# mvenouziou/Boosted_DETR

Measured on AMD Instinct MI355X. Metric: images/sec training step (fwd+matcher+loss+bwd), 640x640 N=100, higher is better.
Workload: dtype f32 (conv/GEMM products as 3 split-f16 [fwd] / split-bf16 [grad] MFMA products, f32 accumulate)

## Files before the change

### boosted_detr_amd/csrc/attention.hip

```cpp
#include "common.h"
#include "p16.h"
#include <stdlib.h>

namespace bdgemm { int gemm_mode(); }

namespace {

typedef unsigned int u32x4 __attribute__((ext_vector_type(4)));
typedef unsigned int u32x2 __attribute__((ext_vector_type(2)));
typedef short s16x4 __attribute__((ext_vector_type(4)));
typedef __bf16 abf16x8 __attribute__((ext_vector_type(8)));
typedef _Float16 af16x8 __attribute__((ext_vector_type(8)));
enum { AR_FP32 = 0, AR_BF16 = 1, AR_F16 = 2 };

constexpr int AD = 32;
constexpr int ALD = AD + 4;
constexpr int CH = 64;
constexpr int COLS_PER_BLOCK = 128;
#ifndef BDETR_ATTN_PF
#define BDETR_ATTN_PF 1
#endif
constexpr int APF = BDETR_ATTN_PF;

constexpr float LOG2E = 1.4426950408889634f, LN2 = 0.6931471805599453f;
__device__ __forceinline__ float exp2_fast(float x) { return __builtin_amdgcn_exp2f(x); }

__device__ __forceinline__ int crow(int e, int lh) { return (e & 3) + 8 * (e >> 2) + 4 * lh; }

struct ChunkRegs { f32x4 v[2]; };
__device__ __forceinline__ ChunkRegs fetch_chunk(const float* __restrict__ base, int64_t stride, int r0, int n) {
    ChunkRegs c;
#pragma unroll
    for (int p = 0; p < 2; ++p) {
        const int v = threadIdx.x + 256 * p;
        const int row = v >> 3, c4 = v & 7;
        const int rr = min(r0 + row, n - 1);
        f32x4 val = *reinterpret_cast<const f32x4*>(base + (int64_t)rr * stride + 4 * c4);
        if (r0 + row >= n) val = f32x4{0.f, 0.f, 0.f, 0.f};
        c.v[p] = val;
    }
    return c;
}
__device__ __forceinline__ void store_chunk(float* __restrict__ lds, const ChunkRegs& c) {
#pragma unroll
    for (int p = 0; p < 2; ++p) {
        const int v = threadIdx.x + 256 * p;
        *reinterpret_cast<f32x4*>(lds + (v >> 3) * ALD + 4 * (v & 7)) = c.v[p];
    }
}

__device__ __forceinline__ void load_col_regs(float (&r)[16], const float* __restrict__ base, int64_t stride, int col, bool ok, int lh) {
#pragma unroll
    for (int c = 0; c < 4; ++c) {
        f32x4 v = {0.f, 0.f, 0.f, 0.f};
        if (ok) v = *reinterpret_cast<const f32x4*>(base + (int64_t)col * stride + 16 * lh + 4 * c);
#pragma unroll
        for (int e = 0; e < 4; ++e) r[4 * c + e] = v[e];
    }
}

__device__ __forceinline__ f32x16 row_times_col(const float* __restrict__ sR, int t, const float (&creg)[16], int li, int lh) {
    f32x16 acc;
#pragma unroll
    for (int e = 0; e < 16; ++e) acc[e] = 0.f;
    f32x4 a[4];
#pragma unroll
    for (int c = 0; c < 4; ++c) a[c] = *reinterpret_cast<const f32x4*>(sR + (32 * t + li) * ALD + 16 * lh + 4 * c);
#pragma unroll
    for (int s = 0; s < 16; ++s) acc = __builtin_amdgcn_mfma_f32_32x32x2f32(a[s >> 2][s & 3], creg[s], acc, 0, 0, 0);
    return acc;
}

__device__ __forceinline__ void accumulate_rt_tile(f32x16& acc, const float* __restrict__ sR, int t, const f32x16& tile, int li, int lh) {
#pragma unroll
    for (int e = 0; e < 16; ++e) {
        const float a = sR[(32 * t + crow(e, lh)) * ALD + li];
        acc = __builtin_amdgcn_mfma_f32_32x32x2f32(a, tile[e], acc, 0, 0, 0);
    }
}

constexpr int IMG_PLANE = CH * 64, IMG_BYTES = 2 * IMG_PLANE;
constexpr int SMEM_BYTES = IMG_BYTES > CH * ALD * 4 ? IMG_BYTES : CH * ALD * 4;

template <int AR>
__device__ __forceinline__ void split2(float x0, float x1, unsigned& hi, unsigned& lo) {
    if (AR == AR_F16) p16_split2_f16(x0, x1, hi, lo); else p16_split2_bf16(x0, x1, hi, lo);
}
template <int AR>
__device__ __forceinline__ f32x16 mfma3(const u32x4& ah, const u32x4& al, const u32x4& bh, const u32x4& bl, f32x16 acc) {
    if (AR == AR_F16) {
#define H8(v) __builtin_bit_cast(af16x8, v)
        acc = __builtin_amdgcn_mfma_f32_32x32x16_f16(H8(al), H8(bh), acc, 0, 0, 0);
        acc = __builtin_amdgcn_mfma_f32_32x32x16_f16(H8(ah), H8(bl), acc, 0, 0, 0);
        acc = __builtin_amdgcn_mfma_f32_32x32x16_f16(H8(ah), H8(bh), acc, 0, 0, 0);
#undef H8
    } else {
#define B8(v) __builtin_bit_cast(abf16x8, v)
        acc = __builtin_amdgcn_mfma_f32_32x32x16_bf16(B8(al), B8(bh), acc, 0, 0, 0);
        acc = __builtin_amdgcn_mfma_f32_32x32x16_bf16(B8(ah), B8(bl), acc, 0, 0, 0);
        acc = __builtin_amdgcn_mfma_f32_32x32x16_bf16(B8(ah), B8(bh), acc, 0, 0, 0);
#undef B8
    }
    return acc;
}
template <int AR>
__device__ __forceinline__ void store_chunk_split(unsigned char* __restrict__ img, const ChunkRegs& c) {
#pragma unroll
    for (int p = 0; p < 2; ++p) {
        const int v = threadIdx.x + 256 * p, row = v >> 3, c4 = v & 7;
        unsigned h0, l0, h1, l1;
        split2<AR>(c.v[p][0], c.v[p][1], h0, l0);
        split2<AR>(c.v[p][2], c.v[p][3], h1, l1);
        const int off = row * 64 + (((c4 >> 1) ^ ((row >> 2) & 3)) << 4) + ((c4 & 1) << 3);
        *reinterpret_cast<u32x2*>(img + off) = u32x2{h0, h1};
        *reinterpret_cast<u32x2*>(img + IMG_PLANE + off) = u32x2{l0, l1};
    }
}
struct ColFrag { u32x4 h[2], l[2]; };
template <int AR>
__device__ __forceinline__ ColFrag col_frag(const float (&r)[16]) {
    ColFrag f;
#pragma unroll
    for (int s2 = 0; s2 < 2; ++s2)
#pragma unroll
        for (int e = 0; e < 4; ++e) { unsigned h, l; split2<AR>(r[8 * s2 + 2 * e], r[8 * s2 + 2 * e + 1], h, l); f.h[s2][e] = h; f.l[s2][e] = l; }
    return f;
}
template <int AR>
__device__ __forceinline__ f32x16 row_times_col_split(const unsigned char* __restrict__ img, int t, const ColFrag& c, int li, int lh) {
    f32x16 acc;
#pragma unroll
    for (int e = 0; e < 16; ++e) acc[e] = 0.f;
    const int row = 32 * t + li;
#pragma unroll
    for (int s2 = 0; s2 < 2; ++s2) {
        const int off = row * 64 + (((2 * lh + s2) ^ ((row >> 2) & 3)) << 4);
        const u32x4 ah = *reinterpret_cast<const u32x4*>(img + off), al = *reinterpret_cast<const u32x4*>(img + IMG_PLANE + off);
        acc = mfma3<AR>(ah, al, c.h[s2], c.l[s2], acc);
    }
    return acc;
}
template <int AR>
__device__ __forceinline__ void accumulate_rt_tile_split(f32x16& acc, const unsigned char* __restrict__ img, int t, const f32x16& tile, int lane) {
    const int lh = lane >> 5, g16 = (lane >> 4) & 1, q = (lane >> 2) & 3, p = lane & 3;
#pragma unroll
    for (int s2 = 0; s2 < 2; ++s2) {
        u32x4 bh, bl;
#pragma unroll
        for (int e = 0; e < 4; ++e) { unsigned h, l; split2<AR>(tile[8 * s2 + 2 * e], tile[8 * s2 + 2 * e + 1], h, l); bh[e] = h; bl[e] = l; }
        u32x2 ah2[2], al2[2];
#pragma unroll
        for (int jj = 0; jj < 2; ++jj) {
            const int row = 32 * t + 16 * s2 + 8 * jj + 4 * lh + q;
            const int off = row * 64 + ((((2 * g16) + (p >> 1)) ^ ((row >> 2) & 3)) << 4) + ((p & 1) << 3);
            ah2[jj] = __builtin_bit_cast(u32x2, __builtin_amdgcn_ds_read_tr16_b64_v4i16((__attribute__((address_space(3))) s16x4*)(img + off)));
            al2[jj] = __builtin_bit_cast(u32x2, __builtin_amdgcn_ds_read_tr16_b64_v4i16((__attribute__((address_space(3))) s16x4*)(img + IMG_PLANE + off)));
        }
        const u32x4 ah = {ah2[0][0], ah2[0][1], ah2[1][0], ah2[1][1]}, al = {al2[0][0], al2[0][1], al2[1][0], al2[1][1]};
        acc = mfma3<AR>(ah, al, bh, bl, acc);
    }
}

template <int AR> struct ColOperand { float r[16]; ColFrag f; };
template <int AR>
__device__ __forceinline__ void chunk_store(unsigned char* smem, const ChunkRegs& c) {
    if constexpr (AR == AR_FP32) store_chunk(reinterpret_cast<float*>(smem), c); else store_chunk_split<AR>(smem, c);
}
template <int AR>
__device__ __forceinline__ f32x16 rows_x_col(const unsigned char* smem, int t, const ColOperand<AR>& c, int li, int lh) {
    if constexpr (AR == AR_FP32) return row_times_col(reinterpret_cast<const float*>(smem), t, c.r, li, lh);
    else return row_times_col_split<AR>(smem, t, c.f, li, lh);
}
template <int AR>
__device__ __forceinline__ void rowsT_x_tile(f32x16& acc, const unsigned char* smem, int t, const f32x16& tile, int lane) {
    if constexpr (AR == AR_FP32) accumulate_rt_tile(acc, reinterpret_cast<const float*>(smem), t, tile, lane & 31, lane >> 5);
    else accumulate_rt_tile_split<AR>(acc, smem, t, tile, lane);
}
template <int AR>
__device__ __forceinline__ void col_operand(ColOperand<AR>& c, const float* __restrict__ base, int64_t stride, int col, bool ok, int lh) {
    load_col_regs(c.r, base, stride, col, ok, lh);
    if constexpr (AR != AR_FP32) c.f = col_frag<AR>(c.r);
}

template <int AR>
__global__ __launch_bounds__(256) void attn_fwd_kernel(const float* __restrict__ q, const float* __restrict__ k, const float* __restrict__ v,
                                                       float* __restrict__ o, float* __restrict__ lse,
                                                       int h, int nq, int nk, float scale) {
    __shared__ __attribute__((aligned(16))) unsigned char sK[SMEM_BYTES];
    __shared__ __attribute__((aligned(16))) unsigned char sV[SMEM_BYTES];
    const int b = blockIdx.z, head = blockIdx.y;
    const int lane = threadIdx.x & 63, wave = threadIdx.x >> 6, li = lane & 31, lh = lane >> 5;
    const int64_t D = (int64_t)h * AD;
    const int qi = blockIdx.x * COLS_PER_BLOCK + wave * 32 + li;
    const bool qok = qi < nq;
    ColOperand<AR> qr;
    col_operand<AR>(qr, q + (int64_t)b * nq * D + head * AD, D, qi, qok, lh);
    const float* kbase = k + (int64_t)b * nk * D + head * AD;
    const float* vbase = v + (int64_t)b * nk * D + head * AD;

    f32x16 oacc;
#pragma unroll
    for (int e = 0; e < 16; ++e) oacc[e] = 0.f;
    float m = -INFINITY, l = 0.f;

    const float scale2 = scale * LOG2E;
    const bool wave_active = blockIdx.x * COLS_PER_BLOCK + wave * 32 < nq;
    ChunkRegs ck[APF], cv[APF];
#pragma unroll
    for (int p = 0; p < APF; ++p) {
        ck[p] = ChunkRegs{}; cv[p] = ChunkRegs{};
        if (p * CH < nk) { ck[p] = fetch_chunk(kbase, D, p * CH, nk); cv[p] = fetch_chunk(vbase, D, p * CH, nk); }
    }
    for (int c0 = 0; c0 < nk; c0 += CH) {
        __syncthreads();
        chunk_store<AR>(sK, ck[0]);
        chunk_store<AR>(sV, cv[0]);
        __syncthreads();
#pragma unroll
        for (int p = 0; p + 1 < APF; ++p) { ck[p] = ck[p + 1]; cv[p] = cv[p + 1]; }
        if (c0 + APF * CH < nk) { ck[APF - 1] = fetch_chunk(kbase, D, c0 + APF * CH, nk); cv[APF - 1] = fetch_chunk(vbase, D, c0 + APF * CH, nk); }
        if (!wave_active) continue;
        f32x16 s[2];
        float cmax = -INFINITY;
        const bool full = c0 + CH <= nk;
#pragma unroll
        for (int t = 0; t < 2; ++t) {
            s[t] = rows_x_col<AR>(sK, t, qr, li, lh);
#pragma unroll
            for (int e = 0; e < 16; ++e) s[t][e] *= scale2;
        }
        if (!full) {
#pragma unroll
            for (int t = 0; t < 2; ++t)
#pragma unroll
                for (int e = 0; e < 16; ++e) if (!(c0 + 32 * t + crow(e, lh) < nk)) s[t][e] = -INFINITY;
        }
#pragma unroll
        for (int t = 0; t < 2; ++t)
#pragma unroll
            for (int e = 0; e < 16; ++e) cmax = fmaxf(cmax, s[t][e]);
        cmax = fmaxf(cmax, __shfl_xor(cmax, 32, 64));
        const float mn = fmaxf(m, cmax);
        const float alpha = exp2_fast(m - mn);
        float psum = 0.f;
#pragma unroll
        for (int t = 0; t < 2; ++t)
#pragma unroll
            for (int e = 0; e < 16; ++e) { const float p = exp2_fast(s[t][e] - mn); s[t][e] = p; psum += p; }
        psum += __shfl_xor(psum, 32, 64);
        l = l * alpha + psum;
        m = mn;
#pragma unroll
        for (int e = 0; e < 16; ++e) oacc[e] *= alpha;
#pragma unroll
        for (int t = 0; t < 2; ++t) rowsT_x_tile<AR>(oacc, sV, t, s[t], lane);
    }
    if (qok) {
        const float inv = 1.0f / l;
        float* orow = o + (((int64_t)b * h + head) * nq + qi) * AD;
#pragma unroll
        for (int e = 0; e < 16; ++e) orow[crow(e, lh)] = oacc[e] * inv;
        if (lh == 0) lse[((int64_t)b * h + head) * nq + qi] = m * LN2 + logf(l);
    }
}

__global__ __launch_bounds__(256) void attn_dvec_kernel(const float* __restrict__ o, const float* __restrict__ d_o, float* __restrict__ dvec, int64_t rows) {
    const int64_t row = ((int64_t)blockIdx.x * 256 + threadIdx.x) >> 3;
    const int c4 = threadIdx.x & 7;
    float s = 0.f;
    if (row < rows) {
        const f32x4 a = reinterpret_cast<const f32x4*>(o)[row * 8 + c4], g = reinterpret_cast<const f32x4*>(d_o)[row * 8 + c4];
        s = a[0] * g[0] + a[1] * g[1] + a[2] * g[2] + a[3] * g[3];
    }
    s += __shfl_xor(s, 1, 64); s += __shfl_xor(s, 2, 64); s += __shfl_xor(s, 4, 64);
    if (row < rows && c4 == 0) dvec[row] = s;
}

template <bool KCOL, int AR>
__global__ __launch_bounds__(256) void attn_bwd_kernel(const float* __restrict__ q, const float* __restrict__ k, const float* __restrict__ v,
                                                       const float* __restrict__ d_o, const float* __restrict__ lse, const float* __restrict__ dvec,
                                                       float* __restrict__ out1, float* __restrict__ out2,
                                                       int h, int nq, int nk, float scale) {
    __shared__ __attribute__((aligned(16))) unsigned char sR1[SMEM_BYTES];
    __shared__ __attribute__((aligned(16))) unsigned char sR2[SMEM_BYTES];
    __shared__ float sL[CH], sD[CH];
    const int b = blockIdx.z, head = blockIdx.y;
    const int lane = threadIdx.x & 63, wave = threadIdx.x >> 6, li = lane & 31, lh = lane >> 5;
    const int64_t D = (int64_t)h * AD;
    const int ncol = KCOL ? nk : nq, nrow = KCOL ? nq : nk;
    const int ci = blockIdx.x * COLS_PER_BLOCK + wave * 32 + li;
    const bool cok = ci < ncol;
    const int64_t bh = (int64_t)b * h + head;

    const float* c1base = (KCOL ? k : q) + (int64_t)b * ncol * D + head * AD;
    const float* c2base = KCOL ? (v + (int64_t)b * nk * D + head * AD) : (d_o + bh * nq * AD);
    const int64_t c2stride = KCOL ? D : AD;
    ColOperand<AR> c1r, c2r;
    col_operand<AR>(c1r, c1base, D, ci, cok, lh);
    col_operand<AR>(c2r, c2base, c2stride, ci, cok, lh);
    const float* r1base = (KCOL ? q : k) + (int64_t)b * nrow * D + head * AD;
    const float* r2base = KCOL ? (d_o + bh * nq * AD) : (v + (int64_t)b * nk * D + head * AD);
    const int64_t r2stride = KCOL ? AD : D;

    float Lcol = 0.f, Dcol = 0.f;
    if (!KCOL && cok) { Lcol = lse[bh * nq + ci] * LOG2E; Dcol = dvec[bh * nq + ci]; }
    const float scale2 = scale * LOG2E;

    f32x16 acc1, acc2;
#pragma unroll
    for (int e = 0; e < 16; ++e) { acc1[e] = 0.f; acc2[e] = 0.f; }

    const bool wave_active = blockIdx.x * COLS_PER_BLOCK + wave * 32 < ncol;
    ChunkRegs c1[APF], c2[APF];
#pragma unroll
    for (int p = 0; p < APF; ++p) {
        c1[p] = ChunkRegs{}; c2[p] = ChunkRegs{};
        if (p * CH < nrow) { c1[p] = fetch_chunk(r1base, D, p * CH, nrow); c2[p] = fetch_chunk(r2base, r2stride, p * CH, nrow); }
    }
    for (int c0 = 0; c0 < nrow; c0 += CH) {
        __syncthreads();
        chunk_store<AR>(sR1, c1[0]);
        chunk_store<AR>(sR2, c2[0]);
        if (KCOL && threadIdx.x < CH) {
            const int qi = c0 + threadIdx.x;
            sL[threadIdx.x] = qi < nq ? lse[bh * nq + qi] * LOG2E : 0.f;
            sD[threadIdx.x] = qi < nq ? dvec[bh * nq + qi] : 0.f;
        }
        __syncthreads();
#pragma unroll
        for (int p = 0; p + 1 < APF; ++p) { c1[p] = c1[p + 1]; c2[p] = c2[p + 1]; }
        if (c0 + APF * CH < nrow) { c1[APF - 1] = fetch_chunk(r1base, D, c0 + APF * CH, nrow); c2[APF - 1] = fetch_chunk(r2base, r2stride, c0 + APF * CH, nrow); }
        if (!wave_active) continue;
        const bool full = c0 + CH <= nrow;
#pragma unroll
        for (int t = 0; t < 2; ++t) {
            f32x16 S = rows_x_col<AR>(sR1, t, c1r, li, lh);
            f32x16 G = rows_x_col<AR>(sR2, t, c2r, li, lh);
#pragma unroll
            for (int e = 0; e < 16; ++e) {
                const int r = 32 * t + crow(e, lh);
                const float Lq = KCOL ? sL[r] : Lcol, Dq = KCOL ? sD[r] : Dcol;
                const float p = (full || c0 + r < nrow) ? exp2_fast(S[e] * scale2 - Lq) : 0.f;
                S[e] = p * (G[e] - Dq) * scale;
                G[e] = p;
            }
            rowsT_x_tile<AR>(acc1, sR1, t, S, lane);
            if (KCOL) rowsT_x_tile<AR>(acc2, sR2, t, G, lane);
        }
    }
    if (cok) {
        float* o1 = out1 + ((int64_t)b * ncol + ci) * D + head * AD;
#pragma unroll
        for (int e = 0; e < 16; ++e) o1[crow(e, lh)] = acc1[e];
        if (KCOL) {
            float* o2 = out2 + ((int64_t)b * ncol + ci) * D + head * AD;
#pragma unroll
            for (int e = 0; e < 16; ++e) o2[crow(e, lh)] = acc2[e];
        }
    }
}

bool attn_split_enabled() {
    static int on = -1;
    if (on < 0) { const char* e = getenv("BDETR_ATTN_SPLIT"); on = e ? atoi(e) != 0 : 1; }
    return on != 0;
}

int check_attn(const void* a, const void* b, const void* c, int B, int h, int nq, int nk, const char* who) {
    BDETR_CHECK_ARG(a && b && c, "%s: null pointer", who);
    BDETR_CHECK_ARG(B > 0 && h > 0 && nq > 0 && nk > 0 && B <= 65535 && h <= 65535, "%s: bad sizes B=%d h=%d nq=%d nk=%d", who, B, h, nq, nk);
    BDETR_CHECK_ARG(((uintptr_t)a & 15) == 0 && ((uintptr_t)b & 15) == 0 && ((uintptr_t)c & 15) == 0, "%s: operands must be 16-byte aligned", who);
    return 0;
}

}

extern "C" int bdetr_attention_head_dim(void) { return AD; }

extern "C" int bdetr_attention_fwd(const float* q, const float* k, const float* v, float* o, float* lse,
                                   int B, int h, int nq, int nk, float scale, void* stream) {
    if (int e = check_attn(q, k, v, B, h, nq, nk, "bdetr_attention_fwd")) return e;
    BDETR_CHECK_ARG(o && lse, "bdetr_attention_fwd: null output");
    dim3 grid((nq + COLS_PER_BLOCK - 1) / COLS_PER_BLOCK, h, B);
    const int mode = attn_split_enabled() ? bdgemm::gemm_mode() : BDETR_GEMM_FP32;
    if (mode == BDETR_GEMM_SPLIT) hipLaunchKernelGGL((attn_fwd_kernel<AR_F16>), grid, dim3(256), 0, (hipStream_t)stream, q, k, v, o, lse, h, nq, nk, scale);
    else if (mode == BDETR_GEMM_BF16X3) hipLaunchKernelGGL((attn_fwd_kernel<AR_BF16>), grid, dim3(256), 0, (hipStream_t)stream, q, k, v, o, lse, h, nq, nk, scale);
    else hipLaunchKernelGGL((attn_fwd_kernel<AR_FP32>), grid, dim3(256), 0, (hipStream_t)stream, q, k, v, o, lse, h, nq, nk, scale);
    return bdetr_launch_status("attention_fwd");
}

extern "C" int bdetr_attention_bwd(const float* q, const float* k, const float* v, const float* o, const float* d_o,
                                   const float* lse, float* dq, float* dk, float* dv, float* dvec_ws,
                                   int B, int h, int nq, int nk, float scale, void* stream) {
    if (int e = check_attn(q, k, v, B, h, nq, nk, "bdetr_attention_bwd")) return e;
    BDETR_CHECK_ARG(o && d_o && lse && dq && dk && dv && dvec_ws, "bdetr_attention_bwd: null pointer");
    hipStream_t st = (hipStream_t)stream;
    const int64_t rows = (int64_t)B * h * nq;
    hipLaunchKernelGGL(attn_dvec_kernel, dim3((unsigned)((rows * 8 + 255) / 256)), dim3(256), 0, st, o, d_o, dvec_ws, rows);
    const dim3 gq((nq + COLS_PER_BLOCK - 1) / COLS_PER_BLOCK, h, B), gk((nk + COLS_PER_BLOCK - 1) / COLS_PER_BLOCK, h, B);
    if (!attn_split_enabled() || bdgemm::gemm_mode() == BDETR_GEMM_FP32 || bdgemm::gemm_mode() == BDETR_GEMM_BF16X6) {
        hipLaunchKernelGGL((attn_bwd_kernel<false, AR_FP32>), gq, dim3(256), 0, st, q, k, v, d_o, lse, dvec_ws, dq, (float*)nullptr, h, nq, nk, scale);
        hipLaunchKernelGGL((attn_bwd_kernel<true, AR_FP32>), gk, dim3(256), 0, st, q, k, v, d_o, lse, dvec_ws, dk, dv, h, nq, nk, scale);
    } else {
        hipLaunchKernelGGL((attn_bwd_kernel<false, AR_BF16>), gq, dim3(256), 0, st, q, k, v, d_o, lse, dvec_ws, dq, (float*)nullptr, h, nq, nk, scale);
        hipLaunchKernelGGL((attn_bwd_kernel<true, AR_BF16>), gk, dim3(256), 0, st, q, k, v, d_o, lse, dvec_ws, dk, dv, h, nq, nk, scale);
    }
    return bdetr_launch_status("attention_bwd");
}
```

Baseline: 660.1.

## Adapt attention block size to grid, fuse dvec into dQ backward, skip empty half-chunks

```diff
diff --git a/boosted_detr_amd/csrc/attention.hip b/boosted_detr_amd/csrc/attention.hip
--- a/boosted_detr_amd/csrc/attention.hip
+++ b/boosted_detr_amd/csrc/attention.hip
@@ -2,7 +2,7 @@
 #include "p16.h"
 #include <stdlib.h>
 
-namespace bdgemm { int gemm_mode(); }
+namespace bdgemm { int gemm_mode(); int num_cus(); }
 
 namespace {
 
@@ -16,7 +16,6 @@
 constexpr int AD = 32;
 constexpr int ALD = AD + 4;
 constexpr int CH = 64;
-constexpr int COLS_PER_BLOCK = 128;
 #ifndef BDETR_ATTN_PF
 #define BDETR_ATTN_PF 1
 #endif
@@ -27,12 +26,13 @@
 
 __device__ __forceinline__ int crow(int e, int lh) { return (e & 3) + 8 * (e >> 2) + 4 * lh; }
 
-struct ChunkRegs { f32x4 v[2]; };
-__device__ __forceinline__ ChunkRegs fetch_chunk(const float* __restrict__ base, int64_t stride, int r0, int n) {
-    ChunkRegs c;
-#pragma unroll
-    for (int p = 0; p < 2; ++p) {
-        const int v = threadIdx.x + 256 * p;
+template <int NW> struct ChunkRegs { f32x4 v[8 / NW]; };
+template <int NW>
+__device__ __forceinline__ ChunkRegs<NW> fetch_chunk(const float* __restrict__ base, int64_t stride, int r0, int n) {
+    ChunkRegs<NW> c;
+#pragma unroll
+    for (int p = 0; p < 8 / NW; ++p) {
+        const int v = threadIdx.x + 64 * NW * p;
         const int row = v >> 3, c4 = v & 7;
         const int rr = min(r0 + row, n - 1);
         f32x4 val = *reinterpret_cast<const f32x4*>(base + (int64_t)rr * stride + 4 * c4);
@@ -41,10 +41,11 @@
     }
     return c;
 }
-__device__ __forceinline__ void store_chunk(float* __restrict__ lds, const ChunkRegs& c) {
-#pragma unroll
-    for (int p = 0; p < 2; ++p) {
-        const int v = threadIdx.x + 256 * p;
+template <int NW>
+__device__ __forceinline__ void store_chunk(float* __restrict__ lds, const ChunkRegs<NW>& c) {
+#pragma unroll
+    for (int p = 0; p < 8 / NW; ++p) {
+        const int v = threadIdx.x + 64 * NW * p;
         *reinterpret_cast<f32x4*>(lds + (v >> 3) * ALD + 4 * (v & 7)) = c.v[p];
     }
 }
@@ -103,11 +104,11 @@
     }
     return acc;
 }
-template <int AR>
-__device__ __forceinline__ void store_chunk_split(unsigned char* __restrict__ img, const ChunkRegs& c) {
-#pragma unroll
-    for (int p = 0; p < 2; ++p) {
-        const int v = threadIdx.x + 256 * p, row = v >> 3, c4 = v & 7;
+template <int AR, int NW>
+__device__ __forceinline__ void store_chunk_split(unsigned char* __restrict__ img, const ChunkRegs<NW>& c) {
+#pragma unroll
+    for (int p = 0; p < 8 / NW; ++p) {
+        const int v = threadIdx.x + 64 * NW * p, row = v >> 3, c4 = v & 7;
         unsigned h0, l0, h1, l1;
         split2<AR>(c.v[p][0], c.v[p][1], h0, l0);
         split2<AR>(c.v[p][2], c.v[p][3], h1, l1);
@@ -162,9 +163,9 @@
 }
 
 template <int AR> struct ColOperand { float r[16]; ColFrag f; };
-template <int AR>
-__device__ __forceinline__ void chunk_store(unsigned char* smem, const ChunkRegs& c) {
-    if constexpr (AR == AR_FP32) store_chunk(reinterpret_cast<float*>(smem), c); else store_chunk_split<AR>(smem, c);
+template <int AR, int NW>
+__device__ __forceinline__ void chunk_store(unsigned char* smem, const ChunkRegs<NW>& c) {
+    if constexpr (AR == AR_FP32) store_chunk<NW>(reinterpret_cast<float*>(smem), c); else store_chunk_split<AR, NW>(smem, c);
 }
 template <int AR>
 __device__ __forceinline__ f32x16 rows_x_col(const unsigned char* smem, int t, const ColOperand<AR>& c, int li, int lh) {
@@ -182,16 +183,16 @@
     if constexpr (AR != AR_FP32) c.f = col_frag<AR>(c.r);
 }
 
-template <int AR>
-__global__ __launch_bounds__(256) void attn_fwd_kernel(const float* __restrict__ q, const float* __restrict__ k, const float* __restrict__ v,
-                                                       float* __restrict__ o, float* __restrict__ lse,
-                                                       int h, int nq, int nk, float scale) {
+template <int AR, int NW>
+__global__ __launch_bounds__(64 * NW) void attn_fwd_kernel(const float* __restrict__ q, const float* __restrict__ k, const float* __restrict__ v,
+                                                           float* __restrict__ o, float* __restrict__ lse,
+                                                           int h, int nq, int nk, float scale) {
     __shared__ __attribute__((aligned(16))) unsigned char sK[SMEM_BYTES];
     __shared__ __attribute__((aligned(16))) unsigned char sV[SMEM_BYTES];
     const int b = blockIdx.z, head = blockIdx.y;
     const int lane = threadIdx.x & 63, wave = threadIdx.x >> 6, li = lane & 31, lh = lane >> 5;
     const int64_t D = (int64_t)h * AD;
-    const int qi = blockIdx.x * COLS_PER_BLOCK + wave * 32 + li;
+    const int q0 = (blockIdx.x * NW + wave) * 32, qi = q0 + li;
     const bool qok = qi < nq;
     ColOperand<AR> qr;
     col_operand<AR>(qr, q + (int64_t)b * nq * D + head * AD, D, qi, qok, lh);
@@ -204,39 +205,25 @@
     float m = -INFINITY, l = 0.f;
 
     const float scale2 = scale * LOG2E;
-    const bool wave_active = blockIdx.x * COLS_PER_BLOCK + wave * 32 < nq;
-    ChunkRegs ck[APF], cv[APF];
-#pragma unroll
-    for (int p = 0; p < APF; ++p) {
-        ck[p] = ChunkRegs{}; cv[p] = ChunkRegs{};
-        if (p * CH < nk) { ck[p] = fetch_chunk(kbase, D, p * CH, nk); cv[p] = fetch_chunk(vbase, D, p * CH, nk); }
-    }
-    for (int c0 = 0; c0 < nk; c0 += CH) {
-        __syncthreads();
-        chunk_store<AR>(sK, ck[0]);
-        chunk_store<AR>(sV, cv[0]);
-        __syncthreads();
-#pragma unroll
-        for (int p = 0; p + 1 < APF; ++p) { ck[p] = ck[p + 1]; cv[p] = cv[p + 1]; }
-        if (c0 + APF * CH < nk) { ck[APF - 1] = fetch_chunk(kbase, D, c0 + APF * CH, nk); cv[APF - 1] = fetch_chunk(vbase, D, c0 + APF * CH, nk); }
-        if (!wave_active) continue;
-        f32x16 s[2];
+    const bool wave_active = q0 < nq;
+    auto chunk = [&]<int NT>(int c0) {
+        f32x16 s[NT];
         float cmax = -INFINITY;
         const bool full = c0 + CH <= nk;
 #pragma unroll
-        for (int t = 0; t < 2; ++t) {
+        for (int t = 0; t < NT; ++t) {
             s[t] = rows_x_col<AR>(sK, t, qr, li, lh);
 #pragma unroll
             for (int e = 0; e < 16; ++e) s[t][e] *= scale2;
         }
         if (!full) {
 #pragma unroll
-            for (int t = 0; t < 2; ++t)
+            for (int t = 0; t < NT; ++t)
 #pragma unroll
                 for (int e = 0; e < 16; ++e) if (!(c0 + 32 * t + crow(e, lh) < nk)) s[t][e] = -INFINITY;
         }
 #pragma unroll
-        for (int t = 0; t < 2; ++t)
+        for (int t = 0; t < NT; ++t)
 #pragma unroll
             for (int e = 0; e < 16; ++e) cmax = fmaxf(cmax, s[t][e]);
         cmax = fmaxf(cmax, __shfl_xor(cmax, 32, 64));
@@ -244,7 +231,7 @@
         const float alpha = exp2_fast(m - mn);
         float psum = 0.f;
 #pragma unroll
-        for (int t = 0; t < 2; ++t)
+        for (int t = 0; t < NT; ++t)
 #pragma unroll
             for (int e = 0; e < 16; ++e) { const float p = exp2_fast(s[t][e] - mn); s[t][e] = p; psum += p; }
         psum += __shfl_xor(psum, 32, 64);
@@ -253,7 +240,24 @@
 #pragma unroll
         for (int e = 0; e < 16; ++e) oacc[e] *= alpha;
 #pragma unroll
-        for (int t = 0; t < 2; ++t) rowsT_x_tile<AR>(oacc, sV, t, s[t], lane);
+        for (int t = 0; t < NT; ++t) rowsT_x_tile<AR>(oacc, sV, t, s[t], lane);
+    };
+    ChunkRegs<NW> ck[APF], cv[APF];
+#pragma unroll
+    for (int p = 0; p < APF; ++p) {
+        ck[p] = ChunkRegs<NW>{}; cv[p] = ChunkRegs<NW>{};
+        if (p * CH < nk) { ck[p] = fetch_chunk<NW>(kbase, D, p * CH, nk); cv[p] = fetch_chunk<NW>(vbase, D, p * CH, nk); }
+    }
+    for (int c0 = 0; c0 < nk; c0 += CH) {
+        __syncthreads();
+        chunk_store<AR, NW>(sK, ck[0]);
+        chunk_store<AR, NW>(sV, cv[0]);
+        __syncthreads();
+#pragma unroll
+        for (int p = 0; p + 1 < APF; ++p) { ck[p] = ck[p + 1]; cv[p] = cv[p + 1]; }
+        if (c0 + APF * CH < nk) { ck[APF - 1] = fetch_chunk<NW>(kbase, D, c0 + APF * CH, nk); cv[APF - 1] = fetch_chunk<NW>(vbase, D, c0 + APF * CH, nk); }
+        if (!wave_active) continue;
+        if (c0 + 32 < nk) chunk.template operator()<2>(c0); else chunk.template operator()<1>(c0);
     }
     if (qok) {
         const float inv = 1.0f / l;
@@ -264,23 +268,11 @@
     }
 }
 
-__global__ __launch_bounds__(256) void attn_dvec_kernel(const float* __restrict__ o, const float* __restrict__ d_o, float* __restrict__ dvec, int64_t rows) {
-    const int64_t row = ((int64_t)blockIdx.x * 256 + threadIdx.x) >> 3;
-    const int c4 = threadIdx.x & 7;
-    float s = 0.f;
-    if (row < rows) {
-        const f32x4 a = reinterpret_cast<const f32x4*>(o)[row * 8 + c4], g = reinterpret_cast<const f32x4*>(d_o)[row * 8 + c4];
-        s = a[0] * g[0] + a[1] * g[1] + a[2] * g[2] + a[3] * g[3];
-    }
-    s += __shfl_xor(s, 1, 64); s += __shfl_xor(s, 2, 64); s += __shfl_xor(s, 4, 64);
-    if (row < rows && c4 == 0) dvec[row] = s;
-}
-
-template <bool KCOL, int AR>
-__global__ __launch_bounds__(256) void attn_bwd_kernel(const float* __restrict__ q, const float* __restrict__ k, const float* __restrict__ v,
-                                                       const float* __restrict__ d_o, const float* __restrict__ lse, const float* __restrict__ dvec,
-                                                       float* __restrict__ out1, float* __restrict__ out2,
-                                                       int h, int nq, int nk, float scale) {
+template <bool KCOL, int AR, int NW>
+__global__ __launch_bounds__(64 * NW) void attn_bwd_kernel(const float* __restrict__ q, const float* __restrict__ k, const float* __restrict__ v,
+                                                           const float* __restrict__ o, const float* __restrict__ d_o, const float* __restrict__ lse,
+                                                           float* __restrict__ dvec, float* __restrict__ out1, float* __restrict__ out2,
+                                                           int h, int nq, int nk, float scale) {
     __shared__ __attribute__((aligned(16))) unsigned char sR1[SMEM_BYTES];
     __shared__ __attribute__((aligned(16))) unsigned char sR2[SMEM_BYTES];
     __shared__ float sL[CH], sD[CH];
@@ -288,7 +280,7 @@
     const int lane = threadIdx.x & 63, wave = threadIdx.x >> 6, li = lane & 31, lh = lane >> 5;
     const int64_t D = (int64_t)h * AD;
     const int ncol = KCOL ? nk : nq, nrow = KCOL ? nq : nk;
-    const int ci = blockIdx.x * COLS_PER_BLOCK + wave * 32 + li;
+    const int col0 = (blockIdx.x * NW + wave) * 32, ci = col0 + li;
     const bool cok = ci < ncol;
     const int64_t bh = (int64_t)b * h + head;
 
@@ -303,37 +295,28 @@
     const int64_t r2stride = KCOL ? AD : D;
 
     float Lcol = 0.f, Dcol = 0.f;
-    if (!KCOL && cok) { Lcol = lse[bh * nq + ci] * LOG2E; Dcol = dvec[bh * nq + ci]; }
+    if constexpr (!KCOL) {
+        float orow[16];
+        load_col_regs(orow, o + bh * nq * AD, AD, ci, cok, lh);
+#pragma unroll
+        for (int s = 0; s < 16; ++s) Dcol += c2r.r[s] * orow[s];
+        Dcol += __shfl_xor(Dcol, 32, 64);
+        if (cok) {
+            Lcol = lse[bh * nq + ci] * LOG2E;
+            if (lh == 0) dvec[bh * nq + ci] = Dcol;
+        }
+    }
     const float scale2 = scale * LOG2E;
 
     f32x16 acc1, acc2;
 #pragma unroll
     for (int e = 0; e < 16; ++e) { acc1[e] = 0.f; acc2[e] = 0.f; }
 
-    const bool wave_active = blockIdx.x * COLS_PER_BLOCK + wave * 32 < ncol;
-    ChunkRegs c1[APF], c2[APF];
-#pragma unroll
-    for (int p = 0; p < APF; ++p) {
-        c1[p] = ChunkRegs{}; c2[p] = ChunkRegs{};
-        if (p * CH < nrow) { c1[p] = fetch_chunk(r1base, D, p * CH, nrow); c2[p] = fetch_chunk(r2base, r2stride, p * CH, nrow); }
-    }
-    for (int c0 = 0; c0 < nrow; c0 += CH) {
-        __syncthreads();
-        chunk_store<AR>(sR1, c1[0]);
-        chunk_store<AR>(sR2, c2[0]);
-        if (KCOL && threadIdx.x < CH) {
-            const int qi = c0 + threadIdx.x;
-            sL[threadIdx.x] = qi < nq ? lse[bh * nq + qi] * LOG2E : 0.f;
-            sD[threadIdx.x] = qi < nq ? dvec[bh * nq + qi] : 0.f;
-        }
-        __syncthreads();
-#pragma unroll
-        for (int p = 0; p + 1 < APF; ++p) { c1[p] = c1[p + 1]; c2[p] = c2[p + 1]; }
-        if (c0 + APF * CH < nrow) { c1[APF - 1] = fetch_chunk(r1base, D, c0 + APF * CH, nrow); c2[APF - 1] = fetch_chunk(r2base, r2stride, c0 + APF * CH, nrow); }
-        if (!wave_active) continue;
+    const bool wave_active = col0 < ncol;
+    auto chunk = [&]<int NT>(int c0) {
         const bool full = c0 + CH <= nrow;
 #pragma unroll
-        for (int t = 0; t < 2; ++t) {
+        for (int t = 0; t < NT; ++t) {
             f32x16 S = rows_x_col<AR>(sR1, t, c1r, li, lh);
             f32x16 G = rows_x_col<AR>(sR2, t, c2r, li, lh);
 #pragma unroll
@@ -347,6 +330,28 @@
             rowsT_x_tile<AR>(acc1, sR1, t, S, lane);
             if (KCOL) rowsT_x_tile<AR>(acc2, sR2, t, G, lane);
         }
+    };
+    ChunkRegs<NW> c1[APF], c2[APF];
+#pragma unroll
+    for (int p = 0; p < APF; ++p) {
+        c1[p] = ChunkRegs<NW>{}; c2[p] = ChunkRegs<NW>{};
+        if (p * CH < nrow) { c1[p] = fetch_chunk<NW>(r1base, D, p * CH, nrow); c2[p] = fetch_chunk<NW>(r2base, r2stride, p * CH, nrow); }
+    }
+    for (int c0 = 0; c0 < nrow; c0 += CH) {
+        __syncthreads();
+        chunk_store<AR, NW>(sR1, c1[0]);
+        chunk_store<AR, NW>(sR2, c2[0]);
+        if (KCOL && threadIdx.x < CH) {
+            const int qi = c0 + threadIdx.x;
+            sL[threadIdx.x] = qi < nq ? lse[bh * nq + qi] * LOG2E : 0.f;
+            sD[threadIdx.x] = qi < nq ? dvec[bh * nq + qi] : 0.f;
+        }
+        __syncthreads();
+#pragma unroll
+        for (int p = 0; p + 1 < APF; ++p) { c1[p] = c1[p + 1]; c2[p] = c2[p + 1]; }
+        if (c0 + APF * CH < nrow) { c1[APF - 1] = fetch_chunk<NW>(r1base, D, c0 + APF * CH, nrow); c2[APF - 1] = fetch_chunk<NW>(r2base, r2stride, c0 + APF * CH, nrow); }
+        if (!wave_active) continue;
+        if (c0 + 32 < nrow) chunk.template operator()<2>(c0); else chunk.template operator()<1>(c0);
     }
     if (cok) {
         float* o1 = out1 + ((int64_t)b * ncol + ci) * D + head * AD;
@@ -364,6 +369,16 @@
     static int on = -1;
     if (on < 0) { const char* e = getenv("BDETR_ATTN_SPLIT"); on = e ? atoi(e) != 0 : 1; }
     return on != 0;
+}
+
+int attn_waves(int ncol, int64_t bh) {
+    static int forced = -1;
+    if (forced < 0) { const char* e = getenv("BDETR_ATTN_TILE"); forced = e ? atoi(e) : 0; }
+    if (forced == 32 || forced == 64 || forced == 128) return forced / 32;
+    const int64_t tiles = cdiv64(ncol, 32);
+    for (int nw = 4; nw > 1; nw >>= 1)
+        if (cdiv64(tiles, nw) * nw - tiles <= 1 && cdiv64(tiles, nw) * bh >= 2 * bdgemm::num_cus()) return nw;
+    return 1;
 }
 
 int check_attn(const void* a, const void* b, const void* c, int B, int h, int nq, int nk, const char* who) {
@@ -373,6 +388,33 @@
     return 0;
 }
 
+template <int AR, int NW>
+void launch_fwd(const float* q, const float* k, const float* v, float* o, float* lse, int B, int h, int nq, int nk, float scale, hipStream_t st) {
+    hipLaunchKernelGGL((attn_fwd_kernel<AR, NW>), dim3((nq + 32 * NW - 1) / (32 * NW), h, B), dim3(64 * NW), 0, st, q, k, v, o, lse, h, nq, nk, scale);
+}
+template <int AR>
+void launch_fwd(int nw, const float* q, const float* k, const float* v, float* o, float* lse, int B, int h, int nq, int nk, float scale, hipStream_t st) {
+    if (nw == 4) launch_fwd<AR, 4>(q, k, v, o, lse, B, h, nq, nk, scale, st);
+    else if (nw == 2) launch_fwd<AR, 2>(q, k, v, o, lse, B, h, nq, nk, scale, st);
+    else launch_fwd<AR, 1>(q, k, v, o, lse, B, h, nq, nk, scale, st);
+}
+
+template <bool KCOL, int AR, int NW>
+void launch_bwd(const float* q, const float* k, const float* v, const float* o, const float* d_o, const float* lse, float* dvec, float* out1, float* out2,
+                int B, int h, int nq, int nk, float scale, hipStream_t st) {
+    const int ncol = KCOL ? nk : nq;
+    hipLaunchKernelGGL((attn_bwd_kernel<KCOL, AR, NW>), dim3((ncol + 32 * NW - 1) / (32 * NW), h, B), dim3(64 * NW), 0, st,
+                       q, k, v, o, d_o, lse, dvec, out1, out2, h, nq, nk, scale);
+}
+template <bool KCOL, int AR>
+void launch_bwd(const float* q, const float* k, const float* v, const float* o, const float* d_o, const float* lse, float* dvec, float* out1, float* out2,
+                int B, int h, int nq, int nk, float scale, hipStream_t st) {
+    const int nw = attn_waves(KCOL ? nk : nq, (int64_t)B * h);
+    if (nw == 4) launch_bwd<KCOL, AR, 4>(q, k, v, o, d_o, lse, dvec, out1, out2, B, h, nq, nk, scale, st);
+    else if (nw == 2) launch_bwd<KCOL, AR, 2>(q, k, v, o, d_o, lse, dvec, out1, out2, B, h, nq, nk, scale, st);
+    else launch_bwd<KCOL, AR, 1>(q, k, v, o, d_o, lse, dvec, out1, out2, B, h, nq, nk, scale, st);
+}
+
 }
 
 extern "C" int bdetr_attention_head_dim(void) { return AD; }
@@ -381,11 +423,12 @@
                                    int B, int h, int nq, int nk, float scale, void* stream) {
     if (int e = check_attn(q, k, v, B, h, nq, nk, "bdetr_attention_fwd")) return e;
     BDETR_CHECK_ARG(o && lse, "bdetr_attention_fwd: null output");
-    dim3 grid((nq + COLS_PER_BLOCK - 1) / COLS_PER_BLOCK, h, B);
+    hipStream_t st = (hipStream_t)stream;
+    const int nw = attn_waves(nq, (int64_t)B * h);
     const int mode = attn_split_enabled() ? bdgemm::gemm_mode() : BDETR_GEMM_FP32;
-    if (mode == BDETR_GEMM_SPLIT) hipLaunchKernelGGL((attn_fwd_kernel<AR_F16>), grid, dim3(256), 0, (hipStream_t)stream, q, k, v, o, lse, h, nq, nk, scale);
-    else if (mode == BDETR_GEMM_BF16X3) hipLaunchKernelGGL((attn_fwd_kernel<AR_BF16>), grid, dim3(256), 0, (hipStream_t)stream, q, k, v, o, lse, h, nq, nk, scale);
-    else hipLaunchKernelGGL((attn_fwd_kernel<AR_FP32>), grid, dim3(256), 0, (hipStream_t)stream, q, k, v, o, lse, h, nq, nk, scale);
+    if (mode == BDETR_GEMM_SPLIT) launch_fwd<AR_F16>(nw, q, k, v, o, lse, B, h, nq, nk, scale, st);
+    else if (mode == BDETR_GEMM_BF16X3) launch_fwd<AR_BF16>(nw, q, k, v, o, lse, B, h, nq, nk, scale, st);
+    else launch_fwd<AR_FP32>(nw, q, k, v, o, lse, B, h, nq, nk, scale, st);
     return bdetr_launch_status("attention_fwd");
 }
 
@@ -395,15 +438,12 @@
     if (int e = check_attn(q, k, v, B, h, nq, nk, "bdetr_attention_bwd")) return e;
     BDETR_CHECK_ARG(o && d_o && lse && dq && dk && dv && dvec_ws, "bdetr_attention_bwd: null pointer");
     hipStream_t st = (hipStream_t)stream;
-    const int64_t rows = (int64_t)B * h * nq;
-    hipLaunchKernelGGL(attn_dvec_kernel, dim3((unsigned)((rows * 8 + 255) / 256)), dim3(256), 0, st, o, d_o, dvec_ws, rows);
-    const dim3 gq((nq + COLS_PER_BLOCK - 1) / COLS_PER_BLOCK, h, B), gk((nk + COLS_PER_BLOCK - 1) / COLS_PER_BLOCK, h, B);
     if (!attn_split_enabled() || bdgemm::gemm_mode() == BDETR_GEMM_FP32 || bdgemm::gemm_mode() == BDETR_GEMM_BF16X6) {
-        hipLaunchKernelGGL((attn_bwd_kernel<false, AR_FP32>), gq, dim3(256), 0, st, q, k, v, d_o, lse, dvec_ws, dq, (float*)nullptr, h, nq, nk, scale);
-        hipLaunchKernelGGL((attn_bwd_kernel<true, AR_FP32>), gk, dim3(256), 0, st, q, k, v, d_o, lse, dvec_ws, dk, dv, h, nq, nk, scale);
+        launch_bwd<false, AR_FP32>(q, k, v, o, d_o, lse, dvec_ws, dq, nullptr, B, h, nq, nk, scale, st);
+        launch_bwd<true, AR_FP32>(q, k, v, o, d_o, lse, dvec_ws, dk, dv, B, h, nq, nk, scale, st);
     } else {
-        hipLaunchKernelGGL((attn_bwd_kernel<false, AR_BF16>), gq, dim3(256), 0, st, q, k, v, d_o, lse, dvec_ws, dq, (float*)nullptr, h, nq, nk, scale);
-        hipLaunchKernelGGL((attn_bwd_kernel<true, AR_BF16>), gk, dim3(256), 0, st, q, k, v, d_o, lse, dvec_ws, dk, dv, h, nq, nk, scale);
+        launch_bwd<false, AR_BF16>(q, k, v, o, d_o, lse, dvec_ws, dq, nullptr, B, h, nq, nk, scale, st);
+        launch_bwd<true, AR_BF16>(q, k, v, o, d_o, lse, dvec_ws, dk, dv, B, h, nq, nk, scale, st);
     }
     return bdetr_launch_status("attention_bwd");
 }
```

After: 657.1. About the same (-0.5%).
